# LarsELund/Bayesian-Neural-Nets

Hardware: AMD Instinct MI355X
Metric: ELBO forward samples/sec, 784-1200^2-10 MNF MLP, batch 4096 per GPU (higher is better)
Workload: dtype f16 (row-scaled fp16 hi + lo split of the f32 operands: 3 mean + 1 variance MFMA products, f32 accumulate)

## Files before the change

### bayesian-neural-nets_amd/csrc/lbbnn_internal.h

```cpp
#pragma once
#include <hip/hip_runtime.h>
#include <stdint.h>
#include "../../include/lbbnn.h"
#include "lbbnn_device.h"

namespace lbbnn {

#define LBBNN_HIDDEN __attribute__((visibility("hidden")))

struct WeightPassArgs {
    const float* mu; const float* rho; const float* lambdal;
    const float* z_fwd; const float* z_kl; const float* r0_c; const float* bias_rho;
    float* e_w; float* var_w;
    float* kl_rows; float* act_mu; float* act_var; float* bias_var;
    int O, I, ld, vec;
    int split;
    float* e_scale; float* v_scale;
    float mu_prior, sigma_prior, alpha_prior;
    float log_sp, log_ap, log_1map, inv_2sp2;
};

struct FlowArgs {
    const float* q0_mean; const float* q0_log_var;
    const float* eps_fwd; const float* eps_kl;
// ... 33 lines not shown
        else dst = (arr)[3];                                   \
    } while (0)
static_assert(LBBNN_MAX_LAYERS == 4, "LBBNN_SELECT_LAYER enumerates 4 layers");

inline bool off(const void* p, uintptr_t n) { return (reinterpret_cast<uintptr_t>(p) & (n - 1)) != 0; }
inline bool aligned16(const void* p) { return !off(p, 16); }
inline bool aligned4(const void* p) { return !off(p, 4); }

LBBNN_HIDDEN int make_weight_pass_args(WeightPassArgs& a, const float* mu, const float* rho, const float* lambdal,
                                       const float* z_fwd, const float* z_kl, const float* r0_c, const float* bias_rho,
                                       const lbbnn_priors_t* priors, void* e_w, void* var_w, int ld,
                                       float* kl_rows, float* act_mu, float* act_var, float* bias_var, int O, int I,
                                       int split = 0, float* e_scale = nullptr, float* v_scale = nullptr);
LBBNN_HIDDEN int launch_weight_pass(const WeightPassArgs* a, int n, hipStream_t s, uint64_t* rng = nullptr,
                                    uint64_t* rng_snap = nullptr, uint64_t advance = 0, const InFlow* flows = nullptr,
                                    int members = 1);
LBBNN_HIDDEN bool in_flow_eligible(const FlowArgs& f, const WeightPassArgs& w);
LBBNN_HIDDEN void make_in_flow(InFlow& o, const FlowArgs& f);
LBBNN_HIDDEN int launch_flow_planar(const FlowArgs* a, int n, hipStream_t s, int members = 1, unsigned long long m_adv = 0,
                                    long long z_ms = 0, const struct FormatJob* fmt = nullptr, bool* fmt_done = nullptr);
LBBNN_HIDDEN int launch_kl_finalize_all(const FinalizeArgs* a, const int* active, int n, uint64_t* rng, uint64_t advance,
                                        float* kl_total, hipStream_t s);
LBBNN_HIDDEN int launch_kl_finalize(const FinalizeArgs* a, int n, hipStream_t s);
LBBNN_HIDDEN int fill_finalize_args(const lbbnn_layer_desc_t* L, int n, const uint64_t* rng, FinalizeArgs* ka, int* active);

}
```

### bayesian-neural-nets_amd/csrc/mnf_flow.hip

```cpp
#include <cstdlib>
#include "lbbnn_device.h"
#include "lbbnn_internal.h"

namespace {

using namespace lbbnn;

typedef lbbnn_planar_flow_t PlanarSet;
struct FlowBatch { FlowArgs l[LBBNN_MAX_LAYERS];
                   unsigned long long m_adv; long long z_ms;
                   FormatJob fmt; int fmt_blocks; };
struct FinalizeBatch { FinalizeArgs l[LBBNN_MAX_LAYERS]; };

__device__ __forceinline__ float planar_apply(const PlanarSet& ps, float* z, int I, double* scratch) {
    float logdet = 0.f;
    for (int t = 0; t < ps.T; ++t) {
        const float* __restrict__ u = ps.u[t];
        const float* __restrict__ w = ps.w[t];
        double s_wz = 0.0, s_uw = 0.0;
        for (int i = threadIdx.x; i < I; i += 256) {
            const float wi = w[i];
            s_wz += (double)(wi * z[i]);
            s_uw += (double)(u[i] * wi);
        }
        s_wz = block_sum<double, 4>(s_wz, scratch);
        s_uw = block_sum<double, 4>(s_uw, scratch);
// ... 253 lines not shown
        if (klblk && i == I - 1) {
#pragma unroll
            for (int t = 0; t < kFastT; ++t) if (t >= Tz && t < NT) v += uw[(2 * t) * P + i] * th[t];
            a.scal[3] = v;
        }
    }
    if (tid == 0) {
        if (!klblk) { if (a.scal) a.scal[4] = ld_q; }
        else { a.scal[0] = ld_q; a.scal[1] = (float)acc[NV - 1]; a.scal[2] = ld_r; }
    }
}

constexpr int kVecThreads = 512;

__global__ __launch_bounds__(kVecThreads) void mnf_flow_planar_vec_kernel(const FlowBatch bt) {
    if (blockIdx.x >= 2) {
        if (blockIdx.y == 0 && blockIdx.z == 0)
            format_x_items(bt.fmt, (size_t)(blockIdx.x - 2) * kVecThreads + threadIdx.x, (size_t)bt.fmt_blocks * kVecThreads);
        return;
    }
    const LBBNN_CONST_AS FlowArgs& a = kernarg_as<FlowBatch>()->l[blockIdx.y];
    const bool klblk = blockIdx.x == 1;
    if (klblk && !a.want_kl) return;
    constexpr int NV = 2 * kFastT + kFastT * (kFastT - 1) / 2 + 1;
    constexpr int NW = kVecThreads / 64;
    __shared__ float red[NV][NW];
    const int I = a.I, nq = I >> 2, tid = threadIdx.x, lane = tid & 63, wv = tid >> 6;
    const bool on = tid < nq;
    const float* eps = klblk ? a.eps_kl : a.eps_fwd;
    const int Tz = a.zf.T, Tr = klblk ? a.rf.T : 0, NT = Tz + Tr;
    const float4 zero4 = make_float4(0.f, 0.f, 0.f, 0.f);
    float4 qm = zero4, lv = zero4, ep = zero4, u[kFastT], w[kFastT];
    float bias[kFastT];
#pragma unroll
    for (int t = 0; t < kFastT; ++t) { u[t] = zero4; w[t] = zero4; bias[t] = 0.f; }
// ... 362 lines not shown

bool fill_set(PlanarSet& ps, const float* const* u, const float* const* w, const float* const* b, int T) {
    ps.T = T;
    for (int t = 0; t < LBBNN_MAX_FLOW_T; ++t) { ps.u[t] = nullptr; ps.w[t] = nullptr; ps.b[t] = nullptr; }
    for (int t = 0; t < T; ++t) {
        if (!u || !w || !b || !u[t] || !w[t] || !b[t]) return false;
        ps.u[t] = u[t]; ps.w[t] = w[t]; ps.b[t] = b[t];
    }
    return true;
}

}

namespace lbbnn {

int launch_flow_planar(const FlowArgs* a, int n, hipStream_t s, int members, unsigned long long m_adv, long long z_ms,
                       const FormatJob* fmt, bool* fmt_done) {
    FlowBatch bt;
    bt.m_adv = m_adv; bt.z_ms = z_ms;
    bt.fmt = FormatJob{}; bt.fmt_blocks = 0;
    if (fmt_done) *fmt_done = false;
    int maxI = 0; bool small_t = true, any_kl = false;
    for (int i = 0; i < n; ++i) {
        bt.l[i] = a[i];
        maxI = a[i].I > maxI ? a[i].I : maxI;
        any_kl = any_kl || a[i].want_kl;
    }
    const dim3 grid(any_kl ? 2 : 1, n, members > 1 ? members : 1), block(256);
    (void)small_t;
    size_t need = 0;
    for (int i = 0; i < n; ++i) {
        const size_t v = (size_t)(4 + 2 * (a[i].zf.T + (a[i].want_kl ? a[i].rf.T : 0))) * pad64(a[i].I) * sizeof(float);
        need = v > need ? v : need;
    }
    if (need <= (size_t)kFlowLdsBudget) {
        if (need > 64 * 1024) {
// ... 5 lines not shown
            if (e != hipSuccess) return (int)e;
        }
        bool fast = true;
        for (int i = 0; i < n; ++i) fast = fast && (a[i].zf.T + (a[i].want_kl ? a[i].rf.T : 0) <= kFastT);
        static const bool vec_allowed = [] { const char* e = getenv("LBBNN_K3_VEC"); return !(e && e[0] == '0'); }();
        bool vec = fast && vec_allowed;
        auto al16 = [](const void* p) { return (reinterpret_cast<uintptr_t>(p) & 15u) == 0; };
        for (int i = 0; i < n && vec; ++i) {
            const FlowArgs& f = a[i];
            vec = (f.I % 4 == 0) && f.I <= 4 * kVecThreads && al16(f.q0_mean) && al16(f.q0_log_var) && al16(f.z_fwd) &&
                  (!f.eps_fwd || al16(f.eps_fwd)) && (!f.want_kl || (al16(f.z_kl) && (!f.eps_kl || al16(f.eps_kl)))) &&
                  (z_ms % 4 == 0);
            for (int t = 0; t < f.zf.T && vec; ++t) vec = al16(f.zf.u[t]) && al16(f.zf.w[t]);
            for (int t = 0; t < (f.want_kl ? f.rf.T : 0) && vec; ++t) vec = al16(f.rf.u[t]) && al16(f.rf.w[t]);
        }
        if (vec && fmt && fmt->x && any_kl) {
            const size_t items = (size_t)fmt->B * (fmt->ldp >> 3);
            bt.fmt = *fmt;
            bt.fmt_blocks = (int)((items + kVecThreads - 1) / kVecThreads < 1024 ? (items + kVecThreads - 1) / kVecThreads : 1024);
            dim3 g2(2 + bt.fmt_blocks, n, grid.z);
            hipLaunchKernelGGL(mnf_flow_planar_vec_kernel, g2, dim3(kVecThreads), 0, s, bt);
            if (fmt_done) *fmt_done = true;
        } else if (vec) hipLaunchKernelGGL(mnf_flow_planar_vec_kernel, grid, dim3(kVecThreads), 0, s, bt);
        else if (fast) hipLaunchKernelGGL(mnf_flow_planar_fast_kernel, grid, dim3(kFastThreads), need, s, bt);
        else if (members > 1) return LBBNN_E_SHAPE;
        else      hipLaunchKernelGGL(mnf_flow_planar_lds_kernel, grid, block, need, s, bt);
    } else {
        if (members > 1) return LBBNN_E_SHAPE;
        hipLaunchKernelGGL(mnf_flow_planar_kernel, grid, block, (size_t)maxI * sizeof(float), s, bt);
    }
    return (int)hipGetLastError();
}

int launch_kl_finalize_all(const FinalizeArgs* a, const int* active, int n, uint64_t* rng, uint64_t advance, float* kl_total,
                           hipStream_t s) {
    FinalizeAllArgs fa;
    for (int i = 0; i < LBBNN_MAX_LAYERS; ++i) { fa.l[i] = i < n ? a[i] : FinalizeArgs{}; fa.active[i] = i < n ? active[i] : 0; }
    fa.n = n; fa.rng = rng; fa.advance = advance; fa.total = kl_total;
// ... 138 lines not shown
```

### bayesian-neural-nets_amd/csrc/prepare.hip

```cpp
#include <cstdlib>
#include "lbbnn_internal.h"

using namespace lbbnn;

static int layers_prepare_impl(const lbbnn_layer_desc_t* L, int n, const uint64_t* rng, void* stream, bool with_k5,
                               uint64_t* rng_live = nullptr, uint64_t* rng_snap = nullptr, uint64_t advance = 0,
                               const FormatJob* fmt = nullptr) {
    if (!L) return LBBNN_E_NULL;
    if (n <= 0 || n > LBBNN_MAX_LAYERS) return LBBNN_E_SHAPE;
    FlowArgs fa[LBBNN_MAX_LAYERS];
    WeightPassArgs wa[LBBNN_MAX_LAYERS];
    FinalizeArgs ka[LBBNN_MAX_LAYERS];
    int flow_of[LBBNN_MAX_LAYERS];
    int nf = 0, nk = 0;
    for (int i = 0; i < n; ++i) {
        const lbbnn_layer_desc_t& d = L[i];
        const bool mnf = d.q0_mean != nullptr;
        flow_of[i] = -1;
        if (!d.weight_mu || !d.weight_rho || !d.lambdal || !d.bias_mu || !d.bias_rho || !d.e_w || !d.bias_var) return LBBNN_E_NULL;
        if (d.stochastic && !d.var_w) return LBBNN_E_NULL;
        if (d.want_kl && (!d.kl_rows || !d.kl_layer)) return LBBNN_E_NULL;
        if (mnf && d.flows_done) {
            if (!d.z_fwd || (d.want_kl && (!d.z_kl || !d.scal || !d.r0_c || !d.r0_b1 || !d.r0_b2 || !d.act_mu || !d.act_var))) return LBBNN_E_NULL;
        } else if (mnf) {
// ... 29 lines not shown
            k.bias_mu_prior = d.priors.bias_mu_prior; k.bias_sigma_prior = d.priors.bias_sigma_prior;
        }
    }
    hipStream_t s = static_cast<hipStream_t>(stream);
    int rc = 0;
    InFlow inf[LBBNN_MAX_LAYERS] = {};
    static const bool inflow_allowed = [] { const char* e = getenv("LBBNN_K1_INFLOW"); return e && e[0] == '1'; }();
    bool in_kernel = nf > 0 && advance == 0 && inflow_allowed;
    for (int i = 0; i < n && in_kernel; ++i) {
        in_kernel = wa[i].vec && wa[i].ld <= 2048;
        if (in_kernel && flow_of[i] >= 0) in_kernel = in_flow_eligible(fa[flow_of[i]], wa[i]);
    }
    if (in_kernel) {
        for (int i = 0; i < n; ++i) if (flow_of[i] >= 0) make_in_flow(inf[i], fa[flow_of[i]]);
    } else if (nf) {
        bool fmt_done = false;
        rc = launch_flow_planar(fa, nf, s, 1, 0, 0, fmt, &fmt_done); if (rc) return rc;
        if (fmt_done) fmt = nullptr;
    }
    if (fmt) {
        rc = lbbnn_format_x(fmt->x, fmt->ldx, fmt->planes, fmt->ldp, fmt->B, fmt->I, stream); if (rc) return rc;
    }
    rc = launch_weight_pass(wa, n, s, rng_live, rng_snap, advance, in_kernel ? inf : nullptr); if (rc) return rc;
    if (nk && with_k5) { rc = launch_kl_finalize(ka, nk, s); if (rc) return rc; }
    return 0;
}

extern "C" int lbbnn_layers_prepare(const lbbnn_layer_desc_t* L, int n, const uint64_t* rng, void* stream) {
    return layers_prepare_impl(L, n, rng, stream, true);
}

extern "C" int lbbnn_layers_operands(const lbbnn_layer_desc_t* L, int n, const uint64_t* rng, void* stream) {
    return layers_prepare_impl(L, n, rng, stream, false);
}

extern "C" int lbbnn_layers_operands_snap(const lbbnn_layer_desc_t* L, int n, uint64_t* rng, uint64_t* rng_snap,
                                          uint64_t advance, void* stream) {
    if (rng && !rng_snap) return LBBNN_E_NULL;
// ... 94 lines not shown
```

### bayesian-neural-nets_amd/csrc/weight_pass.hip

```cpp
#include <cmath>
#include <cstdlib>
#include "lbbnn_device.h"
#include "lbbnn_internal.h"
#include "operand_store.h"

namespace {

using namespace lbbnn;

struct WeightPassBatch { WeightPassArgs l[LBBNN_MAX_LAYERS]; int row_end[LBBNN_MAX_LAYERS]; int n;
                         uint64_t* rng; uint64_t* rng_snap; uint64_t advance; };

struct Elem { float ew, vw, kl, amu, avar; };

typedef float k1_floatx2 __attribute__((ext_vector_type(2)));
typedef _Float16 k1_f16x2 __attribute__((ext_vector_type(2)));
__device__ __forceinline__ uint32_t cvt_pk_h(float a, float b) {
    const k1_floatx2 v = {a, b};
    return __builtin_bit_cast(uint32_t, __builtin_convertvector(v, k1_f16x2));
}
__device__ __forceinline__ void split4_h(const float4 w, uint2& hi, uint2& lo) {
    const uint32_t h0 = cvt_pk_h(w.x, w.y), h1 = cvt_pk_h(w.z, w.w);
    const k1_f16x2 f0 = __builtin_bit_cast(k1_f16x2, h0), f1 = __builtin_bit_cast(k1_f16x2, h1);
    hi = make_uint2(h0, h1);
// ... 201 lines not shown
        const k1_f2 one_m = 1.f - alpha;
        const k1_f2 t = ((c.log_sp - lsig) - 0.5f) + (la - c.log_ap) + fma2(d, d, s2) * c.inv_2sp2;
        e.kl = alpha * t + one_m * (l1m - c.log_1map);
    }
    if (want_act) {
        e.amu = rc * ((zk * mu) * alpha);
        e.avar = (rc * rc) * e.vw;
    }
    return e;
}

constexpr int kInT = 4;
constexpr int kInNV = 3 * kInT + kInT * (kInT - 1) / 2 + kInT + 1;
constexpr int kRowG = 8;
constexpr int kRowB = 5;
#ifndef LBBNN_K1_ROWS_PER_WG
#define LBBNN_K1_ROWS_PER_WG 1
#endif
constexpr int kRowsWGFlow = 4;
constexpr int kRowsWG = LBBNN_K1_ROWS_PER_WG;
template <bool INFLOW> struct RowsCfg { static constexpr int RW = INFLOW ? kRowsWGFlow : kRowsWG, NT = 64 * RW; };

struct WeightRowsBatch {
    WeightPassArgs l[LBBNN_MAX_LAYERS];
    InFlow f[LBBNN_MAX_LAYERS];
    int wg_end[LBBNN_MAX_LAYERS];
    int n;
    uint64_t* rng; uint64_t* rng_snap; uint64_t advance;
    int members;
};

__device__ __forceinline__ float4 ld4(const float* p, int j) { return reinterpret_cast<const float4*>(p)[j]; }
__device__ __forceinline__ float dot4(const float4 a, const float4 b) { return (a.x * b.x + a.y * b.y) + (a.z * b.z + a.w * b.w); }
__device__ __forceinline__ float4 fma4(const float4 u, float s, const float4 z) {
    return make_float4(z.x + u.x * s, z.y + u.y * s, z.z + u.z * s, z.w + u.w * s);
}

template <bool F16S, bool INFLOW>
__global__ __launch_bounds__(RowsCfg<INFLOW>::NT, 3) void weight_rows_kernel(const WeightRowsBatch bt_) {
    constexpr int kRowsWG = RowsCfg<INFLOW>::RW, kRowNT = RowsCfg<INFLOW>::NT;
    const LBBNN_CONST_AS WeightRowsBatch* bt = kernarg_as<WeightRowsBatch>();
    extern __shared__ __attribute__((aligned(16))) float sm[];
    __shared__ double red[INFLOW ? kInNV : 1][kRowsWG];
    const int tid = threadIdx.x, lane = tid & 63, wv = tid >> 6;
    if (bt->rng_snap && blockIdx.x == 0 && tid == 0) {
        const uint64_t sd = bt->rng[0], of = bt->rng[1];
        bt->rng_snap[0] = sd; bt->rng_snap[1] = of;
        if (bt->advance) bt->rng[1] = of + bt->advance;
    }
    int li = 0;
#pragma unroll
    for (int t = 0; t < LBBNN_MAX_LAYERS - 1; ++t) if (t + 1 < bt->n && (int)blockIdx.x >= bt->wg_end[t]) li = t + 1;
    const LBBNN_CONST_AS WeightPassArgs& a = bt->l[li];
    const LBBNN_CONST_AS InFlow& f = bt->f[li];
    const int wg0 = li ? bt->wg_end[li - 1] : 0;
    const bool first_wg = (int)blockIdx.x == wg0;
    const int I = a.I, P = a.ld, nq = P >> 2, iq = I >> 2;
    const int mem = blockIdx.y;
    float* zf_s = sm; float* zk_s = sm + P; float* rc_s = sm + 2 * P;
    const bool want_kl = a.kl_rows != nullptr, want_act = a.act_mu != nullptr;
    const float4 one4 = make_float4(1.f, 1.f, 1.f, 1.f), zero4 = make_float4(0.f, 0.f, 0.f, 0.f);

    const int o = kRowsWG * ((int)blockIdx.x - wg0) + wv;
    const bool has_row = o < a.O;
    const int G = (nq + 63) >> 6;
    const size_t rowoff = (size_t)o * I;

    float4 mu[kRowB], rho[kRowB], lam[kRowB];
    constexpr bool kDirectZ = !INFLOW && kRowsWG == 1;
    float4 zfr[1], zkr[1], rcr[1];
    if (!INFLOW && has_row) {
#pragma unroll
        for (int g = 0; g < kRowB; ++g) {
            const int j = lane + 64 * g;
            if (g < G && j < iq) { mu[g] = ld4(a.mu + rowoff, j); rho[g] = ld4(a.rho + rowoff, j); lam[g] = ld4(a.lambdal + rowoff, j); }
        }
    }
    auto load_z = [&](int gg, float4& zf, float4& zk, float4& rc) {
        const int j = lane + 64 * gg;
        zf = one4; zk = one4; rc = one4;
        if (gg < G && j < iq) {
            if (a.z_fwd) zf = ld4(a.z_fwd + (size_t)mem * P, j);
            if (a.z_kl) zk = ld4(a.z_kl, j);
            if (a.r0_c) rc = ld4(a.r0_c, j);
        }
    };
    if constexpr (kDirectZ) { if (has_row) load_z(0, zfr[0], zkr[0], rcr[0]); }

    if (INFLOW && f.on) {
        const int Tz = f.Tz, NT = f.Tz + f.Tr;
        const bool klb = f.want_kl != 0;
        uint64_t seed = 0, offs = 0;
        if (!f.eps_fwd || (klb && !f.eps_kl)) { seed = f.rng[0]; offs = f.rng[1]; }
        double acc[kInNV];
#pragma unroll
        for (int k = 0; k < kInNV; ++k) acc[k] = 0.0;
#pragma unroll 1
        for (int h = 0; h < 2; ++h) {
            const int j = tid + kRowNT * h;
            if (j < iq) {
                const float4 qm = ld4(f.q0_mean, j), lv = ld4(f.q0_log_var, j);
                float ef[4], ek[4] = {0.f, 0.f, 0.f, 0.f};
                if (f.eps_fwd) { const float4 e = ld4(f.eps_fwd, j); ef[0] = e.x; ef[1] = e.y; ef[2] = e.z; ef[3] = e.w; }
                else philox_normal4(seed, offs, LBBNN_STREAM_EPS_Z * 64u + f.layer, (uint64_t)j, 0u, ef);
// ... 98 lines not shown
                        reinterpret_cast<float4*>(f.z_kl)[j] = zk;
                        if (j == iq - 1) {
                            float v = zk.w;
#pragma unroll
                            for (int t = 0; t < kInT; ++t) if (t >= Tz && t < NT) v += ulast[t] * thk[t];
                            f.scal[3] = v;
                        }
                    }
                }
            }
        }
        if (first_wg && tid == 0 && f.scal) {
            f.scal[4] = ldf;
            if (klb) { f.scal[0] = ldq; f.scal[1] = (float)acc[kInNV - 1]; f.scal[2] = ldr; }
        }
    } else if constexpr (!kDirectZ) {
#pragma unroll
        for (int h = 0; h < (64 * kRowG + kRowNT - 1) / kRowNT; ++h) {
            const int j = tid + kRowNT * h;
            if (j < nq) {
                const bool in = j < iq;
                float4 zf = one4, zk = one4, rc = one4;
                if (a.z_fwd && in) zf = ld4(a.z_fwd + (size_t)mem * P, j);
                if (a.z_kl && in) zk = ld4(a.z_kl, j);
                if (a.r0_c && in) rc = ld4(a.r0_c, j);
                reinterpret_cast<float4*>(zf_s)[j] = zf;
                reinterpret_cast<float4*>(zk_s)[j] = zk;
                reinterpret_cast<float4*>(rc_s)[j] = rc;
            }
        }
    }
    if constexpr (!kDirectZ) __syncthreads();

    if (!has_row) return;
    const ElemConst ec = {a.mu_prior, a.log_sp, a.log_ap, a.log_1map, a.inv_2sp2};
    k1_f2 kl2 = {0.f, 0.f}, amu2 = kl2, avar2 = kl2;
    const bool split = a.split == 1;
    float* const ewp = a.e_w ? a.e_w + (size_t)mem * a.O * P : nullptr;
    float* const vwp = mem == 0 ? a.var_w : nullptr;
    const bool f16s = F16S && a.split >= 2;
    const bool vhi_only = a.split == 3;
    float4 ew_keep[F16S ? kRowB : 1], vw_keep[F16S ? kRowB : 1];
    for (int g0 = 0; g0 < G; g0 += kRowB) {
        if (INFLOW || g0 > 0) {
#pragma unroll
            for (int g = 0; g < kRowB; ++g) {
                const int j = lane + 64 * (g0 + g);
                if (g0 + g < G && j < iq) { mu[g] = ld4(a.mu + rowoff, j); rho[g] = ld4(a.rho + rowoff, j); lam[g] = ld4(a.lambdal + rowoff, j); }
            }
        }
#pragma unroll
        for (int g = 0; g < kRowB; ++g) {
            if (g0 + g >= G) break;
            const int j = lane + 64 * (g0 + g);
            float4 ew = zero4, vw = zero4;
            if constexpr (kDirectZ) { if (g0 + g > 0) load_z(g0 + g, zfr[0], zkr[0], rcr[0]); }
            if (j < iq) {
                float4 zf, zk, rc;
                if constexpr (kDirectZ) { zf = zfr[0]; zk = zkr[0]; rc = rcr[0]; }
                else {
                    zf = reinterpret_cast<const float4*>(zf_s)[j]; zk = reinterpret_cast<const float4*>(zk_s)[j];
                    rc = reinterpret_cast<const float4*>(rc_s)[j];
                }
                const Elem2 ea = weight_elem_p2(k1_f2{mu[g].x, mu[g].y}, k1_f2{rho[g].x, rho[g].y}, k1_f2{lam[g].x, lam[g].y},
                                                k1_f2{zf.x, zf.y}, k1_f2{zk.x, zk.y}, k1_f2{rc.x, rc.y}, want_kl, want_act, ec);
                const Elem2 eb = weight_elem_p2(k1_f2{mu[g].z, mu[g].w}, k1_f2{rho[g].z, rho[g].w}, k1_f2{lam[g].z, lam[g].w},
                                                k1_f2{zf.z, zf.w}, k1_f2{zk.z, zk.w}, k1_f2{rc.z, rc.w}, want_kl, want_act, ec);
                ew = make_float4(ea.ew.x, ea.ew.y, eb.ew.x, eb.ew.y);
                vw = make_float4(ea.vw.x, ea.vw.y, eb.vw.x, eb.vw.y);
                kl2 += ea.kl + eb.kl;
                amu2 += ea.amu + eb.amu;
                avar2 += ea.avar + eb.avar;
            }
            if constexpr (F16S) {
                ew_keep[g] = ew; vw_keep[g] = vw;
            } else if (!split) {
                if (j < nq) {
                    if (ewp) reinterpret_cast<float4*>(ewp + (size_t)o * P)[j] = ew;
// ... 64 lines not shown
            }
        }
        if (f16s && lane == 0) {
            if (a.e_scale) a.e_scale[o] = ie;
            if (a.v_scale && vwp) a.v_scale[o] = iv;
        }
    }
    if (want_kl || want_act) {
        const float kl = wave_sum(kl2.x + kl2.y), amu = wave_sum(amu2.x + amu2.y), avar = wave_sum(avar2.x + avar2.y);
        if (lane == 0) {
            if (want_kl) a.kl_rows[o] = kl;
            if (want_act) { a.act_mu[o] = amu; a.act_var[o] = avar; }
        }
    }
    if (lane == 0 && mem == 0 && a.bias_var && a.bias_rho) {
        const float sb = softplus_ref(a.bias_rho[o]);
        a.bias_var[o] = sb * sb;
    }
}

}

namespace lbbnn {

int make_weight_pass_args(WeightPassArgs& a, const float* mu, const float* rho, const float* lambdal,
                          const float* z_fwd, const float* z_kl, const float* r0_c, const float* bias_rho,
                          const lbbnn_priors_t* priors, void* e_w, void* var_w, int ld,
                          float* kl_rows, float* act_mu, float* act_var, float* bias_var, int O, int I, int split,
                          float* e_scale, float* v_scale) {
    if (!mu || !rho || !lambdal || !priors) return LBBNN_E_NULL;
// ... 32 lines not shown
               return true;
           }();
}

void make_in_flow(InFlow& o, const FlowArgs& f) {
    o = InFlow{};
    o.on = 1;
    o.q0_mean = f.q0_mean; o.q0_log_var = f.q0_log_var; o.eps_fwd = f.eps_fwd; o.eps_kl = f.want_kl ? f.eps_kl : nullptr;
    o.rng = f.rng; o.z_fwd = f.z_fwd; o.z_kl = f.z_kl; o.scal = f.scal;
    o.Tz = f.zf.T; o.Tr = f.want_kl ? f.rf.T : 0; o.want_kl = f.want_kl; o.layer = f.layer;
    for (int t = 0; t < o.Tz; ++t) { o.u[t] = f.zf.u[t]; o.w[t] = f.zf.w[t]; o.b[t] = f.zf.b[t]; }
    for (int t = 0; t < o.Tr; ++t) { o.u[o.Tz + t] = f.rf.u[t]; o.w[o.Tz + t] = f.rf.w[t]; o.b[o.Tz + t] = f.rf.b[t]; }
}

int launch_weight_pass(const WeightPassArgs* a, int n, hipStream_t s, uint64_t* rng, uint64_t* rng_snap, uint64_t advance,
                       const InFlow* flows, int members) {
    bool rows_ok = true;
    for (int i = 0; i < n; ++i) rows_ok = rows_ok && a[i].vec && a[i].ld <= 64 * 4 * kRowG;
    static const bool rows_allowed = [] { const char* e = getenv("LBBNN_K1_ROWS"); return !(e && e[0] == '0'); }();
    rows_ok = rows_ok && rows_allowed;
    bool any_f16 = false;
    for (int i = 0; i < n; ++i) any_f16 = any_f16 || a[i].split >= 2;
    if (any_f16) {
        for (int i = 0; i < n; ++i) if (!a[i].vec || a[i].ld > 64 * 4 * kRowB) return LBBNN_E_SHAPE;
        if (members > 1) return LBBNN_E_FLAGS;
        rows_ok = true;
    }
    if (rows_ok) {
        WeightRowsBatch bt{};
        bt.rng = rng; bt.rng_snap = (rng && rng_snap) ? rng_snap : nullptr; bt.advance = advance;
        int wgs = 0, maxld = 0;
        bool flow_on = false;
        for (int i = 0; i < n && flows; ++i) flow_on = flow_on || flows[i].on;
        const int rw = flow_on ? RowsCfg<true>::RW : RowsCfg<false>::RW;
        for (int i = 0; i < n; ++i) {
            bt.l[i] = a[i];
            if (flows) bt.f[i] = flows[i];
            if (bt.f[i].on && advance) return LBBNN_E_FLAGS;
            wgs += (a[i].O + rw - 1) / rw; bt.wg_end[i] = wgs;
            maxld = a[i].ld > maxld ? a[i].ld : maxld;
        }
        for (int i = n; i < LBBNN_MAX_LAYERS; ++i) bt.wg_end[i] = wgs;
        bt.n = n;
        bt.members = members;
        if (members > 1) for (int i = 0; i < n; ++i) if (bt.f[i].on || a[i].kl_rows || a[i].act_mu) return LBBNN_E_FLAGS;
        bool any_flow = false;
        for (int i = 0; i < n; ++i) any_flow = any_flow || bt.f[i].on;
        const dim3 grid(wgs, any_f16 ? 1 : (members > 1 ? members : 1));
        const size_t lds = (!flow_on && RowsCfg<false>::RW == 1) ? 0 : (size_t)3 * maxld * sizeof(float);
        if (any_f16 && any_flow)  hipLaunchKernelGGL((weight_rows_kernel<true, true>), grid, dim3(RowsCfg<true>::NT), lds, s, bt);
        else if (any_f16)         hipLaunchKernelGGL((weight_rows_kernel<true, false>), grid, dim3(RowsCfg<false>::NT), lds, s, bt);
        else if (any_flow)        hipLaunchKernelGGL((weight_rows_kernel<false, true>), grid, dim3(RowsCfg<true>::NT), lds, s, bt);
        else                      hipLaunchKernelGGL((weight_rows_kernel<false, false>), grid, dim3(RowsCfg<false>::NT), lds, s, bt);
        return (int)hipGetLastError();
    }
    if (members > 1) return LBBNN_E_ALIGN;
    if (flows) for (int i = 0; i < n; ++i) if (flows[i].on) return LBBNN_E_ALIGN;
    WeightPassBatch bt;
    bt.rng = rng; bt.rng_snap = (rng && rng_snap) ? rng_snap : nullptr; bt.advance = advance;
    int rows = 0;
    for (int i = 0; i < n; ++i) { bt.l[i] = a[i]; rows += a[i].O; bt.row_end[i] = rows; }
    for (int i = n; i < LBBNN_MAX_LAYERS; ++i) bt.row_end[i] = rows;
    bt.n = n;
    hipLaunchKernelGGL(weight_pass_kernel, dim3(rows), dim3(256), 0, s, bt);
    return (int)hipGetLastError();
}

}
// ... 32 lines not shown
```

### bayesian-neural-nets_amd/layers.py

```python
import itertools
import weakref
from typing import Dict, Optional

import torch
import torch.nn as nn
import torch.nn.functional as F

from . import _grad, _lib, ops
from ._lib import Priors
from .distributions import Bernoulli, Gaussian
from .flows import PropagateFlow

import os as _os
_DENSE_HIP_BWD = _os.environ.get("LBBNN_DENSE_TORCH_BWD", "0") != "1"
_MASKS_IN_KERNEL = _os.environ.get("LBBNN_TORCH_MASKS", "0") != "1"
_DENSE_DEFER = {"0": False, "always": "always"}.get(_os.environ.get("LBBNN_DENSE_DEFER", "1"), True)
_HEAD_FOLD = _os.environ.get("LBBNN_HEAD_FOLD", "1") != "0"
_ADV_RIDE = _os.environ.get("LBBNN_ADV_RIDE", "1") != "0"
_V1_BATCH = _os.environ.get("LBBNN_V1_BATCH", "1") != "0"
_DEFER_SUMS = _os.environ.get("LBBNN_DEFER_SUMS", "1") != "0"
_LRT_BIAS_HIP = _os.environ.get("LBBNN_LRT_BIAS_HIP", "1") != "0"
_HEAD_DW = _os.environ.get("LBBNN_HEAD_DW", "1") != "0"
_F16_FIRST_PLANES = _os.environ.get("LBBNN_F16_FIRST", "f32") != "f32"
_SIDE = {}


def _side_stream(dev):
    key = dev.index if dev.index is not None else torch.cuda.current_device()
    st = _SIDE.get(key)
    if st is None:
        st = _SIDE[key] = torch.cuda.Stream(device=dev)
    return st


_OVERLAP = {"on": False, "planar": [], "dense": [], "adopt": [], "sums": []}


def _drop_deferred():
# ... 1120 lines not shown
        for l, c in zip(layers, cfgs):
            if l._mnf and l._check_flows() == "chain":
                noise = l.noise or {}
                eps_z, eps_z2 = noise.get("eps_z"), noise.get("eps_z2")
                if eps_z is not None:
                    eps_z = (eps_z[-1] if eps_z.dim() == 2 else eps_z).contiguous()
                if eps_z2 is not None:
                    eps_z2 = eps_z2.reshape(-1).contiguous()
                keep.extend([eps_z, eps_z2])
                l._chain_flows(rng, eps_z, eps_z2, c[1])
        snap = st.t[2:4] if st is not None else None
        lgroups = _lib.layer_groups(n)
        n0 = lgroups[0][1]
        d0 = _lib.group_slice(descs, 0, n0)
        B, x_planes = x.shape[0], False
        if (layers[0]._split_now >= 2 and _F16_FIRST_PLANES and x.stride(1) == 1 and x.stride(0) % 4 == 0 and x.data_ptr() % 16 == 0
                and B > 0):
            xp = self._planes("in", B, layers[0].in_features, dev, plan)
            _lib.check(_lib.lib().lbbnn_layers_operands_x(d0, n0, rng.data_ptr() if rng is not None else None,
                                                          snap.data_ptr() if snap is not None else None, 0,
                                                          x.data_ptr(), x.stride(0), xp.data_ptr(), xp.stride(0), B,
                                                          layers[0].in_features, stream), "lbbnn_layers_operands_x")
            x, x_planes = xp, True
        else:
            _lib.check(_lib.lib().lbbnn_layers_operands_snap(d0, n0, rng.data_ptr() if rng is not None else None,
                                                             snap.data_ptr() if snap is not None else None, 0, stream),
                       "lbbnn_layers_operands_snap")
        for k, cnt in lgroups[1:]:
            _lib.check(_lib.lib().lbbnn_layers_operands(_lib.group_slice(descs, k, cnt), cnt,
                                                        snap.data_ptr() if snap is not None else None, stream),
                       "lbbnn_layers_operands")
        if deferred is not None:
# ... 102 lines not shown
```

Measured before the change: 33.64 million.

## Move input-format job into new two-wave row-task weight pass kernel

Adds a weight_row_tasks_kernel that processes one weight row per two-wave workgroup, holding z operands in registers instead of LDS. It also appends the x-to-fp16-planes formatting blocks to this kernel's grid rather than to the planar-flow kernel, and removes the old direct-Z single-wave path. The Python side now turns on first-layer planes by default when split==3, so the fused format path runs by default. The aim is better occupancy for the weight pass and launching format work alongside it; the risk is more register pressure and different block balancing.

```diff
diff --git a/bayesian-neural-nets_amd/csrc/lbbnn_internal.h b/bayesian-neural-nets_amd/csrc/lbbnn_internal.h
--- a/bayesian-neural-nets_amd/csrc/lbbnn_internal.h
+++ b/bayesian-neural-nets_amd/csrc/lbbnn_internal.h
@@ -71,11 +71,11 @@
                                        int split = 0, float* e_scale = nullptr, float* v_scale = nullptr);
 LBBNN_HIDDEN int launch_weight_pass(const WeightPassArgs* a, int n, hipStream_t s, uint64_t* rng = nullptr,
                                     uint64_t* rng_snap = nullptr, uint64_t advance = 0, const InFlow* flows = nullptr,
-                                    int members = 1);
+                                    int members = 1, const struct FormatJob* fmt = nullptr, bool* fmt_done = nullptr);
 LBBNN_HIDDEN bool in_flow_eligible(const FlowArgs& f, const WeightPassArgs& w);
 LBBNN_HIDDEN void make_in_flow(InFlow& o, const FlowArgs& f);
 LBBNN_HIDDEN int launch_flow_planar(const FlowArgs* a, int n, hipStream_t s, int members = 1, unsigned long long m_adv = 0,
-                                    long long z_ms = 0, const struct FormatJob* fmt = nullptr, bool* fmt_done = nullptr);
+                                    long long z_ms = 0);
 LBBNN_HIDDEN int launch_kl_finalize_all(const FinalizeArgs* a, const int* active, int n, uint64_t* rng, uint64_t advance,
                                         float* kl_total, hipStream_t s);
 LBBNN_HIDDEN int launch_kl_finalize(const FinalizeArgs* a, int n, hipStream_t s);
diff --git a/bayesian-neural-nets_amd/csrc/mnf_flow.hip b/bayesian-neural-nets_amd/csrc/mnf_flow.hip
--- a/bayesian-neural-nets_amd/csrc/mnf_flow.hip
+++ b/bayesian-neural-nets_amd/csrc/mnf_flow.hip
@@ -8,8 +8,7 @@
 
 typedef lbbnn_planar_flow_t PlanarSet;
 struct FlowBatch { FlowArgs l[LBBNN_MAX_LAYERS];
-                   unsigned long long m_adv; long long z_ms;
-                   FormatJob fmt; int fmt_blocks; };
+                   unsigned long long m_adv; long long z_ms; };
 struct FinalizeBatch { FinalizeArgs l[LBBNN_MAX_LAYERS]; };
 
 __device__ __forceinline__ float planar_apply(const PlanarSet& ps, float* z, int I, double* scratch) {
@@ -293,11 +292,6 @@
 constexpr int kVecThreads = 512;
 
 __global__ __launch_bounds__(kVecThreads) void mnf_flow_planar_vec_kernel(const FlowBatch bt) {
-    if (blockIdx.x >= 2) {
-        if (blockIdx.y == 0 && blockIdx.z == 0)
-            format_x_items(bt.fmt, (size_t)(blockIdx.x - 2) * kVecThreads + threadIdx.x, (size_t)bt.fmt_blocks * kVecThreads);
-        return;
-    }
     const LBBNN_CONST_AS FlowArgs& a = kernarg_as<FlowBatch>()->l[blockIdx.y];
     const bool klblk = blockIdx.x == 1;
     if (klblk && !a.want_kl) return;
@@ -690,12 +684,9 @@
 
 namespace lbbnn {
 
-int launch_flow_planar(const FlowArgs* a, int n, hipStream_t s, int members, unsigned long long m_adv, long long z_ms,
-                       const FormatJob* fmt, bool* fmt_done) {
+int launch_flow_planar(const FlowArgs* a, int n, hipStream_t s, int members, unsigned long long m_adv, long long z_ms) {
     FlowBatch bt;
     bt.m_adv = m_adv; bt.z_ms = z_ms;
-    bt.fmt = FormatJob{}; bt.fmt_blocks = 0;
-    if (fmt_done) *fmt_done = false;
     int maxI = 0; bool small_t = true, any_kl = false;
     for (int i = 0; i < n; ++i) {
         bt.l[i] = a[i];
@@ -731,14 +722,7 @@
             for (int t = 0; t < f.zf.T && vec; ++t) vec = al16(f.zf.u[t]) && al16(f.zf.w[t]);
             for (int t = 0; t < (f.want_kl ? f.rf.T : 0) && vec; ++t) vec = al16(f.rf.u[t]) && al16(f.rf.w[t]);
         }
-        if (vec && fmt && fmt->x && any_kl) {
-            const size_t items = (size_t)fmt->B * (fmt->ldp >> 3);
-            bt.fmt = *fmt;
-            bt.fmt_blocks = (int)((items + kVecThreads - 1) / kVecThreads < 1024 ? (items + kVecThreads - 1) / kVecThreads : 1024);
-            dim3 g2(2 + bt.fmt_blocks, n, grid.z);
-            hipLaunchKernelGGL(mnf_flow_planar_vec_kernel, g2, dim3(kVecThreads), 0, s, bt);
-            if (fmt_done) *fmt_done = true;
-        } else if (vec) hipLaunchKernelGGL(mnf_flow_planar_vec_kernel, grid, dim3(kVecThreads), 0, s, bt);
+        if (vec) hipLaunchKernelGGL(mnf_flow_planar_vec_kernel, grid, dim3(kVecThreads), 0, s, bt);
         else if (fast) hipLaunchKernelGGL(mnf_flow_planar_fast_kernel, grid, dim3(kFastThreads), need, s, bt);
         else if (members > 1) return LBBNN_E_SHAPE;
         else      hipLaunchKernelGGL(mnf_flow_planar_lds_kernel, grid, block, need, s, bt);
diff --git a/bayesian-neural-nets_amd/csrc/prepare.hip b/bayesian-neural-nets_amd/csrc/prepare.hip
--- a/bayesian-neural-nets_amd/csrc/prepare.hip
+++ b/bayesian-neural-nets_amd/csrc/prepare.hip
@@ -67,14 +67,13 @@
     if (in_kernel) {
         for (int i = 0; i < n; ++i) if (flow_of[i] >= 0) make_in_flow(inf[i], fa[flow_of[i]]);
     } else if (nf) {
-        bool fmt_done = false;
-        rc = launch_flow_planar(fa, nf, s, 1, 0, 0, fmt, &fmt_done); if (rc) return rc;
-        if (fmt_done) fmt = nullptr;
+        rc = launch_flow_planar(fa, nf, s); if (rc) return rc;
     }
-    if (fmt) {
+    bool fmt_done = false;
+    rc = launch_weight_pass(wa, n, s, rng_live, rng_snap, advance, in_kernel ? inf : nullptr, 1, fmt, &fmt_done); if (rc) return rc;
+    if (fmt && !fmt_done) {
         rc = lbbnn_format_x(fmt->x, fmt->ldx, fmt->planes, fmt->ldp, fmt->B, fmt->I, stream); if (rc) return rc;
     }
-    rc = launch_weight_pass(wa, n, s, rng_live, rng_snap, advance, in_kernel ? inf : nullptr); if (rc) return rc;
     if (nk && with_k5) { rc = launch_kl_finalize(ka, nk, s); if (rc) return rc; }
     return 0;
 }
diff --git a/bayesian-neural-nets_amd/csrc/weight_pass.hip b/bayesian-neural-nets_amd/csrc/weight_pass.hip
--- a/bayesian-neural-nets_amd/csrc/weight_pass.hip
+++ b/bayesian-neural-nets_amd/csrc/weight_pass.hip
@@ -239,12 +239,7 @@
 constexpr int kInNV = 3 * kInT + kInT * (kInT - 1) / 2 + kInT + 1;
 constexpr int kRowG = 8;
 constexpr int kRowB = 5;
-#ifndef LBBNN_K1_ROWS_PER_WG
-#define LBBNN_K1_ROWS_PER_WG 1
-#endif
 constexpr int kRowsWGFlow = 4;
-constexpr int kRowsWG = LBBNN_K1_ROWS_PER_WG;
-template <bool INFLOW> struct RowsCfg { static constexpr int RW = INFLOW ? kRowsWGFlow : kRowsWG, NT = 64 * RW; };
 
 struct WeightRowsBatch {
     WeightPassArgs l[LBBNN_MAX_LAYERS];
@@ -253,6 +248,7 @@
     int n;
     uint64_t* rng; uint64_t* rng_snap; uint64_t advance;
     int members;
+    FormatJob fmt; int fmt_blocks;
 };
 
 __device__ __forceinline__ float4 ld4(const float* p, int j) { return reinterpret_cast<const float4*>(p)[j]; }
@@ -261,12 +257,12 @@
     return make_float4(z.x + u.x * s, z.y + u.y * s, z.z + u.z * s, z.w + u.w * s);
 }
 
-template <bool F16S, bool INFLOW>
-__global__ __launch_bounds__(RowsCfg<INFLOW>::NT, 3) void weight_rows_kernel(const WeightRowsBatch bt_) {
-    constexpr int kRowsWG = RowsCfg<INFLOW>::RW, kRowNT = RowsCfg<INFLOW>::NT;
+template <bool F16S>
+__global__ __launch_bounds__(64 * kRowsWGFlow, 3) void weight_rows_kernel(const WeightRowsBatch bt_) {
+    constexpr int kRowsWG = kRowsWGFlow, kRowNT = 64 * kRowsWGFlow;
     const LBBNN_CONST_AS WeightRowsBatch* bt = kernarg_as<WeightRowsBatch>();
     extern __shared__ __attribute__((aligned(16))) float sm[];
-    __shared__ double red[INFLOW ? kInNV : 1][kRowsWG];
+    __shared__ double red[kInNV][kRowsWG];
     const int tid = threadIdx.x, lane = tid & 63, wv = tid >> 6;
     if (bt->rng_snap && blockIdx.x == 0 && tid == 0) {
         const uint64_t sd = bt->rng[0], of = bt->rng[1];
@@ -290,29 +286,9 @@
     const bool has_row = o < a.O;
     const int G = (nq + 63) >> 6;
     const size_t rowoff = (size_t)o * I;
-
     float4 mu[kRowB], rho[kRowB], lam[kRowB];
-    constexpr bool kDirectZ = !INFLOW && kRowsWG == 1;
-    float4 zfr[1], zkr[1], rcr[1];
-    if (!INFLOW && has_row) {
-#pragma unroll
-        for (int g = 0; g < kRowB; ++g) {
-            const int j = lane + 64 * g;
-            if (g < G && j < iq) { mu[g] = ld4(a.mu + rowoff, j); rho[g] = ld4(a.rho + rowoff, j); lam[g] = ld4(a.lambdal + rowoff, j); }
-        }
-    }
-    auto load_z = [&](int gg, float4& zf, float4& zk, float4& rc) {
-        const int j = lane + 64 * gg;
-        zf = one4; zk = one4; rc = one4;
-        if (gg < G && j < iq) {
-            if (a.z_fwd) zf = ld4(a.z_fwd + (size_t)mem * P, j);
-            if (a.z_kl) zk = ld4(a.z_kl, j);
-            if (a.r0_c) rc = ld4(a.r0_c, j);
-        }
-    };
-    if constexpr (kDirectZ) { if (has_row) load_z(0, zfr[0], zkr[0], rcr[0]); }
-
-    if (INFLOW && f.on) {
+
+    if (f.on) {
         const int Tz = f.Tz, NT = f.Tz + f.Tr;
         const bool klb = f.want_kl != 0;
         uint64_t seed = 0, offs = 0;
@@ -441,7 +417,7 @@
             f.scal[4] = ldf;
             if (klb) { f.scal[0] = ldq; f.scal[1] = (float)acc[kInNV - 1]; f.scal[2] = ldr; }
         }
-    } else if constexpr (!kDirectZ) {
+    } else {
 #pragma unroll
         for (int h = 0; h < (64 * kRowG + kRowNT - 1) / kRowNT; ++h) {
             const int j = tid + kRowNT * h;
@@ -457,7 +433,7 @@
             }
         }
     }
-    if constexpr (!kDirectZ) __syncthreads();
+    __syncthreads();
 
     if (!has_row) return;
     const ElemConst ec = {a.mu_prior, a.log_sp, a.log_ap, a.log_1map, a.inv_2sp2};
@@ -469,26 +445,19 @@
     const bool vhi_only = a.split == 3;
     float4 ew_keep[F16S ? kRowB : 1], vw_keep[F16S ? kRowB : 1];
     for (int g0 = 0; g0 < G; g0 += kRowB) {
-        if (INFLOW || g0 > 0) {
-#pragma unroll
-            for (int g = 0; g < kRowB; ++g) {
-                const int j = lane + 64 * (g0 + g);
-                if (g0 + g < G && j < iq) { mu[g] = ld4(a.mu + rowoff, j); rho[g] = ld4(a.rho + rowoff, j); lam[g] = ld4(a.lambdal + rowoff, j); }
-            }
+#pragma unroll
+        for (int g = 0; g < kRowB; ++g) {
+            const int j = lane + 64 * (g0 + g);
+            if (g0 + g < G && j < iq) { mu[g] = ld4(a.mu + rowoff, j); rho[g] = ld4(a.rho + rowoff, j); lam[g] = ld4(a.lambdal + rowoff, j); }
         }
 #pragma unroll
         for (int g = 0; g < kRowB; ++g) {
             if (g0 + g >= G) break;
             const int j = lane + 64 * (g0 + g);
             float4 ew = zero4, vw = zero4;
-            if constexpr (kDirectZ) { if (g0 + g > 0) load_z(g0 + g, zfr[0], zkr[0], rcr[0]); }
             if (j < iq) {
-                float4 zf, zk, rc;
-                if constexpr (kDirectZ) { zf = zfr[0]; zk = zkr[0]; rc = rcr[0]; }
-                else {
-                    zf = reinterpret_cast<const float4*>(zf_s)[j]; zk = reinterpret_cast<const float4*>(zk_s)[j];
-                    rc = reinterpret_cast<const float4*>(rc_s)[j];
-                }
+                const float4 zf = reinterpret_cast<const float4*>(zf_s)[j], zk = reinterpret_cast<const float4*>(zk_s)[j],
+                             rc = reinterpret_cast<const float4*>(rc_s)[j];
                 const Elem2 ea = weight_elem_p2(k1_f2{mu[g].x, mu[g].y}, k1_f2{rho[g].x, rho[g].y}, k1_f2{lam[g].x, lam[g].y},
                                                 k1_f2{zf.x, zf.y}, k1_f2{zk.x, zk.y}, k1_f2{rc.x, rc.y}, want_kl, want_act, ec);
                 const Elem2 eb = weight_elem_p2(k1_f2{mu[g].z, mu[g].w}, k1_f2{rho[g].z, rho[g].w}, k1_f2{lam[g].z, lam[g].w},
@@ -583,6 +552,179 @@
         }
     }
     if (lane == 0 && mem == 0 && a.bias_var && a.bias_rho) {
+        const float sb = softplus_ref(a.bias_rho[o]);
+        a.bias_var[o] = sb * sb;
+    }
+}
+
+constexpr int kTaskW = 2;
+constexpr int kTaskWavesEU = 4;
+constexpr int kFmtItemsPerThread = 1;
+constexpr size_t kFmtMaxBlocks = 4096;
+template <bool F16S> struct TaskCfg { static constexpr int NG = ((F16S ? kRowB : kRowG) + kTaskW - 1) / kTaskW; };
+
+template <bool F16S>
+__global__ __launch_bounds__(64 * kTaskW, kTaskWavesEU) void weight_row_tasks_kernel(const WeightRowsBatch bt_) {
+    constexpr int NG = TaskCfg<F16S>::NG;
+    const LBBNN_CONST_AS WeightRowsBatch* bt = kernarg_as<WeightRowsBatch>();
+    __shared__ float mx_s[kTaskW][2];
+    __shared__ k1_f2 part_s[3][64];
+    const int tid = threadIdx.x, lane = tid & 63, wv = tid >> 6;
+    if (bt->rng_snap && blockIdx.x == 0 && tid == 0) {
+        const uint64_t sd = bt->rng[0], of = bt->rng[1];
+        bt->rng_snap[0] = sd; bt->rng_snap[1] = of;
+        if (bt->advance) bt->rng[1] = of + bt->advance;
+    }
+    if ((int)blockIdx.x >= bt->wg_end[LBBNN_MAX_LAYERS - 1]) {
+        const FormatJob fj = {bt->fmt.x, bt->fmt.planes, bt->fmt.ldx, bt->fmt.ldp, bt->fmt.B, bt->fmt.I};
+        format_x_items(fj, (size_t)((int)blockIdx.x - bt->wg_end[LBBNN_MAX_LAYERS - 1]) * (64 * kTaskW) + tid,
+                       (size_t)bt->fmt_blocks * (64 * kTaskW));
+        return;
+    }
+    int li = 0;
+#pragma unroll
+    for (int t = 0; t < LBBNN_MAX_LAYERS - 1; ++t) if (t + 1 < bt->n && (int)blockIdx.x >= bt->wg_end[t]) li = t + 1;
+    const LBBNN_CONST_AS WeightPassArgs& a = bt->l[li];
+    const int o = (int)blockIdx.x - (li ? bt->wg_end[li - 1] : 0);
+    const int I = a.I, P = a.ld, nq = P >> 2, iq = I >> 2;
+    const int mem = blockIdx.y;
+    const bool want_kl = a.kl_rows != nullptr, want_act = a.act_mu != nullptr;
+    const float4 one4 = make_float4(1.f, 1.f, 1.f, 1.f), zero4 = make_float4(0.f, 0.f, 0.f, 0.f);
+    const int G = (nq + 63) >> 6;
+    const int g_lo = wv ? (G + 1) >> 1 : 0, ng = wv ? G >> 1 : (G + 1) >> 1;
+    const size_t rowoff = (size_t)o * I;
+
+    float4 mu[NG], rho[NG], lam[NG], zf[NG], zk[NG], rc[NG];
+#pragma unroll
+    for (int g = 0; g < NG; ++g) {
+        const int j = lane + 64 * (g_lo + g);
+        zf[g] = one4; zk[g] = one4; rc[g] = one4;
+        if (g < ng && j < iq) {
+            mu[g] = ld4(a.mu + rowoff, j); rho[g] = ld4(a.rho + rowoff, j); lam[g] = ld4(a.lambdal + rowoff, j);
+            if (a.z_fwd) zf[g] = ld4(a.z_fwd + (size_t)mem * P, j);
+            if (a.z_kl) zk[g] = ld4(a.z_kl, j);
+            if (a.r0_c) rc[g] = ld4(a.r0_c, j);
+        }
+    }
+    const ElemConst ec = {a.mu_prior, a.log_sp, a.log_ap, a.log_1map, a.inv_2sp2};
+    const k1_f2 zero2 = {0.f, 0.f};
+    k1_f2 kl2 = zero2, amu2 = zero2, avar2 = zero2;
+    k1_f2 tkl[NG], tamu[NG], tavar[NG];
+    float* const ewp = a.e_w ? a.e_w + (size_t)mem * a.O * P : nullptr;
+    float* const vwp = mem == 0 ? a.var_w : nullptr;
+    const bool f16s = F16S && a.split >= 2;
+    const bool vhi_only = a.split == 3;
+    const bool odd = lane & 1;
+    float4 ew_keep[F16S ? NG : 1], vw_keep[F16S ? NG : 1];
+#pragma unroll
+    for (int g = 0; g < NG; ++g) {
+        tkl[g] = zero2; tamu[g] = zero2; tavar[g] = zero2;
+        if (g >= ng) continue;
+        const int j = lane + 64 * (g_lo + g);
+        float4 ew = zero4, vw = zero4;
+        if (j < iq) {
+            const Elem2 ea = weight_elem_p2(k1_f2{mu[g].x, mu[g].y}, k1_f2{rho[g].x, rho[g].y}, k1_f2{lam[g].x, lam[g].y},
+                                            k1_f2{zf[g].x, zf[g].y}, k1_f2{zk[g].x, zk[g].y}, k1_f2{rc[g].x, rc[g].y}, want_kl, want_act, ec);
+            const Elem2 eb = weight_elem_p2(k1_f2{mu[g].z, mu[g].w}, k1_f2{rho[g].z, rho[g].w}, k1_f2{lam[g].z, lam[g].w},
+                                            k1_f2{zf[g].z, zf[g].w}, k1_f2{zk[g].z, zk[g].w}, k1_f2{rc[g].z, rc[g].w}, want_kl, want_act, ec);
+            ew = make_float4(ea.ew.x, ea.ew.y, eb.ew.x, eb.ew.y);
+            vw = make_float4(ea.vw.x, ea.vw.y, eb.vw.x, eb.vw.y);
+            tkl[g] = ea.kl + eb.kl; tamu[g] = ea.amu + eb.amu; tavar[g] = ea.avar + eb.avar;
+        }
+        if (wv == 0) { kl2 = kl2 + tkl[g]; amu2 = amu2 + tamu[g]; avar2 = avar2 + tavar[g]; }
+        if constexpr (F16S) {
+            ew_keep[g] = ew; vw_keep[g] = vw;
+        } else if (a.split != 1) {
+            if (j < nq) {
+                if (ewp) reinterpret_cast<float4*>(ewp + (size_t)o * P)[j] = ew;
+                if (vwp) reinterpret_cast<float4*>(vwp + (size_t)o * P)[j] = vw;
+            }
+        } else {
+            const size_t at = split_hi_index((size_t)o, 4 * (j & ~1), P) + (odd ? kSplitLoOffset : 0);
+            uint2 hi, lo;
+            split4(ew, hi, lo);
+            {
+                const uint4 unit = pair_unit(odd, hi, lo);
+                if (ewp && j < nq) *reinterpret_cast<uint4*>(reinterpret_cast<uint16_t*>(ewp) + at) = unit;
+            }
+            if (vwp) {
+                split4(vw, hi, lo);
+                const uint4 unit = pair_unit(odd, hi, lo);
+                if (j < nq) *reinterpret_cast<uint4*>(reinterpret_cast<uint16_t*>(vwp) + at) = unit;
+            }
+        }
+    }
+    const bool sums = want_kl || want_act;
+    float me = 0.f, mv = 0.f;
+    if constexpr (F16S) {
+        if (f16s) {
+#pragma unroll
+            for (int g = 0; g < NG; ++g) {
+                if (g >= ng) break;
+                me = fmaxf(fmaxf(fmaxf(fmaxf(me, fabsf(ew_keep[g].x)), fabsf(ew_keep[g].y)), fabsf(ew_keep[g].z)), fabsf(ew_keep[g].w));
+                mv = fmaxf(fmaxf(fmaxf(fmaxf(mv, vw_keep[g].x), vw_keep[g].y), vw_keep[g].z), vw_keep[g].w);
+            }
+            me = wave_max(me); mv = wave_max(mv);
+            if (lane == 0) { mx_s[wv][0] = me; mx_s[wv][1] = mv; }
+        }
+    }
+    if (sums && wv == 0) { part_s[0][lane] = kl2; part_s[1][lane] = amu2; part_s[2][lane] = avar2; }
+    if (f16s || sums) __syncthreads();
+    if constexpr (F16S) {
+        float se = 1.f, ie = 1.f, sv = 1.f, iv = 1.f;
+        if (f16s) {
+            me = fmaxf(mx_s[0][0], mx_s[1][0]); mv = fmaxf(mx_s[0][1], mx_s[1][1]);
+            pow2_scale(me, se, ie);
+            pow2_scale(mv, sv, iv);
+        }
+#pragma unroll
+        for (int g = 0; g < NG; ++g) {
+            if (g >= ng) break;
+            const int j = lane + 64 * (g_lo + g);
+            if (a.split == 0) {
+                if (j < nq) {
+                    if (ewp) reinterpret_cast<float4*>(ewp + (size_t)o * P)[j] = ew_keep[g];
+                    if (vwp) reinterpret_cast<float4*>(vwp + (size_t)o * P)[j] = vw_keep[g];
+                }
+                continue;
+            }
+            const size_t at = split_hi_index((size_t)o, 4 * (j & ~1), P) + (odd ? kSplitLoOffset : 0);
+            uint2 hi, lo;
+            {
+                const float4 w = ew_keep[g];
+                if (f16s) split4_hs(w, se, hi, lo);
+                else split4(w, hi, lo);
+                const uint4 unit = pair_unit(odd, hi, lo);
+                if (ewp && j < nq) *reinterpret_cast<uint4*>(reinterpret_cast<uint16_t*>(ewp) + at) = unit;
+            }
+            if (vwp && vhi_only) {
+                const float4 w = vw_keep[g];
+                if (j < nq) *reinterpret_cast<uint2*>(reinterpret_cast<uint16_t*>(vwp) + (size_t)o * P + 4 * j) =
+                    make_uint2(cvt_pk_h(w.x * sv, w.y * sv), cvt_pk_h(w.z * sv, w.w * sv));
+            } else if (vwp) {
+                const float4 w = vw_keep[g];
+                if (f16s) split4_hs(w, sv, hi, lo);
+                else split4(w, hi, lo);
+                const uint4 unit = pair_unit(odd, hi, lo);
+                if (j < nq) *reinterpret_cast<uint4*>(reinterpret_cast<uint16_t*>(vwp) + at) = unit;
+            }
+        }
+        if (f16s && tid == 0) {
+            if (a.e_scale) a.e_scale[o] = ie;
+            if (a.v_scale && vwp) a.v_scale[o] = iv;
+        }
+    }
+    if (sums && wv == kTaskW - 1) {
+        kl2 = part_s[0][lane]; amu2 = part_s[1][lane]; avar2 = part_s[2][lane];
+#pragma unroll
+        for (int g = 0; g < NG; ++g) { kl2 = kl2 + tkl[g]; amu2 = amu2 + tamu[g]; avar2 = avar2 + tavar[g]; }
+        const float kl = wave_sum(kl2.x + kl2.y), amu = wave_sum(amu2.x + amu2.y), avar = wave_sum(avar2.x + avar2.y);
+        if (lane == 0) {
+            if (want_kl) a.kl_rows[o] = kl;
+            if (want_act) { a.act_mu[o] = amu; a.act_var[o] = avar; }
+        }
+    }
+    if (tid == 0 && mem == 0 && a.bias_var && a.bias_rho) {
         const float sb = softplus_ref(a.bias_rho[o]);
         a.bias_var[o] = sb * sb;
     }
@@ -645,7 +787,8 @@
 }
 
 int launch_weight_pass(const WeightPassArgs* a, int n, hipStream_t s, uint64_t* rng, uint64_t* rng_snap, uint64_t advance,
-                       const InFlow* flows, int members) {
+                       const InFlow* flows, int members, const FormatJob* fmt, bool* fmt_done) {
+    if (fmt_done) *fmt_done = false;
     bool rows_ok = true;
     for (int i = 0; i < n; ++i) rows_ok = rows_ok && a[i].vec && a[i].ld <= 64 * 4 * kRowG;
     static const bool rows_allowed = [] { const char* e = getenv("LBBNN_K1_ROWS"); return !(e && e[0] == '0'); }();
@@ -663,7 +806,7 @@
         int wgs = 0, maxld = 0;
         bool flow_on = false;
         for (int i = 0; i < n && flows; ++i) flow_on = flow_on || flows[i].on;
-        const int rw = flow_on ? RowsCfg<true>::RW : RowsCfg<false>::RW;
+        const int rw = flow_on ? kRowsWGFlow : 1;
         for (int i = 0; i < n; ++i) {
             bt.l[i] = a[i];
             if (flows) bt.f[i] = flows[i];
@@ -677,12 +820,23 @@
         if (members > 1) for (int i = 0; i < n; ++i) if (bt.f[i].on || a[i].kl_rows || a[i].act_mu) return LBBNN_E_FLAGS;
         bool any_flow = false;
         for (int i = 0; i < n; ++i) any_flow = any_flow || bt.f[i].on;
-        const dim3 grid(wgs, any_f16 ? 1 : (members > 1 ? members : 1));
-        const size_t lds = (!flow_on && RowsCfg<false>::RW == 1) ? 0 : (size_t)3 * maxld * sizeof(float);
-        if (any_f16 && any_flow)  hipLaunchKernelGGL((weight_rows_kernel<true, true>), grid, dim3(RowsCfg<true>::NT), lds, s, bt);
-        else if (any_f16)         hipLaunchKernelGGL((weight_rows_kernel<true, false>), grid, dim3(RowsCfg<false>::NT), lds, s, bt);
-        else if (any_flow)        hipLaunchKernelGGL((weight_rows_kernel<false, true>), grid, dim3(RowsCfg<true>::NT), lds, s, bt);
-        else                      hipLaunchKernelGGL((weight_rows_kernel<false, false>), grid, dim3(RowsCfg<false>::NT), lds, s, bt);
+        const int ny = any_f16 ? 1 : (members > 1 ? members : 1);
+        if (any_flow) {
+            const dim3 grid(wgs, ny);
+            const size_t lds = (size_t)3 * maxld * sizeof(float);
+            if (any_f16) hipLaunchKernelGGL((weight_rows_kernel<true>), grid, dim3(64 * kRowsWGFlow), lds, s, bt);
+            else         hipLaunchKernelGGL((weight_rows_kernel<false>), grid, dim3(64 * kRowsWGFlow), lds, s, bt);
+            return (int)hipGetLastError();
+        }
+        if (fmt && ny == 1) {
+            const size_t items = (size_t)fmt->B * (fmt->ldp >> 3), per = (size_t)64 * kTaskW * kFmtItemsPerThread;
+            const size_t nb = (items + per - 1) / per;
+            bt.fmt = *fmt; bt.fmt_blocks = (int)(nb < 1 ? 1 : (nb > kFmtMaxBlocks ? kFmtMaxBlocks : nb));
+            if (fmt_done) *fmt_done = true;
+        }
+        const dim3 grid(wgs + bt.fmt_blocks, ny);
+        if (any_f16) hipLaunchKernelGGL((weight_row_tasks_kernel<true>), grid, dim3(64 * kTaskW), 0, s, bt);
+        else         hipLaunchKernelGGL((weight_row_tasks_kernel<false>), grid, dim3(64 * kTaskW), 0, s, bt);
         return (int)hipGetLastError();
     }
     if (members > 1) return LBBNN_E_ALIGN;
diff --git a/bayesian-neural-nets_amd/layers.py b/bayesian-neural-nets_amd/layers.py
--- a/bayesian-neural-nets_amd/layers.py
+++ b/bayesian-neural-nets_amd/layers.py
@@ -21,7 +21,7 @@
 _DEFER_SUMS = _os.environ.get("LBBNN_DEFER_SUMS", "1") != "0"
 _LRT_BIAS_HIP = _os.environ.get("LBBNN_LRT_BIAS_HIP", "1") != "0"
 _HEAD_DW = _os.environ.get("LBBNN_HEAD_DW", "1") != "0"
-_F16_FIRST_PLANES = _os.environ.get("LBBNN_F16_FIRST", "f32") != "f32"
+_F16_FIRST_PLANES = {"f32": False, "planes": True}.get(_os.environ.get("LBBNN_F16_FIRST", ""))
 _SIDE = {}
 
 
@@ -1172,8 +1172,9 @@
         n0 = lgroups[0][1]
         d0 = _lib.group_slice(descs, 0, n0)
         B, x_planes = x.shape[0], False
-        if (layers[0]._split_now >= 2 and _F16_FIRST_PLANES and x.stride(1) == 1 and x.stride(0) % 4 == 0 and x.data_ptr() % 16 == 0
-                and B > 0):
+        first_planes = layers[0]._split_now == 3 if _F16_FIRST_PLANES is None else _F16_FIRST_PLANES
+        if (layers[0]._split_now >= 2 and first_planes and layers[0].in_features % 8 == 0 and x.stride(1) == 1
+                and x.stride(0) % 4 == 0 and x.data_ptr() % 16 == 0 and B > 0):
             xp = self._planes("in", B, layers[0].in_features, dev, plan)
             _lib.check(_lib.lib().lbbnn_layers_operands_x(d0, n0, rng.data_ptr() if rng is not None else None,
                                                           snap.data_ptr() if snap is not None else None, 0,
```

New measurement: 35.47 million, median of 6. +5.4%, better.
